# matt-suncy/symbols-from-video

Hardware: AMD Instinct MI355X
Metric: frames/sec (enc+binarise+dec fwd+bwd), batch 256x256, 1/2/4/8 MI355X (higher is better)
Workload: dtype bf16; 1 GPU; percep_RBVAE fused train step (batch gather from the HBM-resident latent table + fwd+bwd+losses+Adam), item [16,2,8,4,32,32] per GPU = 256 frames/step/GPU (latents of 256x256 frames), latent 32, 4-layer LSTMs, dropout on; parallelism=dp1, graph=True, dist_world_size=1, schedule=one HIP graph per step, devices_visible=1, graphs_captured=1, launcher=torch.distributed.run or self-spawned ranks

## Files before the change

include/rbvae_hip.h:

```cpp
#ifndef RBVAE_HIP_H
#define RBVAE_HIP_H

#include <stddef.h>
#include <stdint.h>

#ifdef __cplusplus
extern "C" {
#endif

#define RBVAE_OK 0
#define RBVAE_E_INVALID (-1)
#define RBVAE_E_LAUNCH (-2)
#define RBVAE_E_UNSUPPORTED (-3)

#define RBVAE_F32 0
#define RBVAE_BF16 1

int rbvae_version(void);
int rbvae_counter_add(unsigned long long* counter, unsigned long long inc, void* stream);
const char* rbvae_last_error(void);

int rbvae_binarize_kl_fwd(const float* h, const float* U, float* y_soft, float* z, float* kl_mean,
                          int rows, int L, float tau, float noise_ratio, float noise_eps, int hard,
                          float kl_p, float kl_eps, int kl_clamp, unsigned long long seed,
// ... 78 lines not shown

int rbvae_pack3(int dtype, const float* in, void* out, int d0, int d1, int d2, long s0, long s1, long s2,
                void* stream);
int rbvae_permute_reduce(const float* in, int nslab, long slab_stride, float* out, int d0, int d1, int d2, long s0,
                         long s1, long s2, float scale, int accumulate, void* stream);
int rbvae_cast_pad(int dtype, const float* in, void* out, int rows, int L, int Lpad, void* stream);
int rbvae_reduce_rows(const float* ws, int rows, int C, float* out, float scale, int accumulate, void* stream);
int rbvae_colsum_partial(int dtype, const void* X, int P, int C, int ld, float* ws, void* stream);
size_t rbvae_colsum_ws_floats(int P, int C);
int rbvae_colsum(int dtype, const void* X, int P, int C, int ld, float* out, float* ws, float scale, int accumulate,
                 void* stream);

int rbvae_run_jobs(const void* jobs_dev, int njobs, int blocks_per_job, void* stream);
int rbvae_job_block_map(const long* rows_host, int njobs, int max_blocks_per_job, int* map_host, int map_capacity);
int rbvae_run_jobs_sized(const void* jobs_dev, const void* block_map_dev, int total_blocks, void* stream);

int rbvae_im2col(int dtype, const float* src, long sn, long sc, long sh, long sw, int N, int C, int IH, int IW,
                 int OH, int OW, int KH, int KW, int stride, int pad, int Kpad, void* col, void* stream);
int rbvae_conv_first_fused_ok(int dtype, int Cin, int IH, int IW, int Nout, int N);
int rbvae_conv_first_fused(int dtype, const float* x, int fd1, int fd2, long fs0, long fs1, long fs2, const void* W,
                           const float* bias, const void* zero_page, void* col, void* out, int N, int Cin, int IH, int IW,
                           int Nout, int ldo, int relu, int drop_mode, float drop_p, float scale, unsigned long long seed,
                           const unsigned long long* seed_dev, void* stream);
int rbvae_deconv_last_dgrad_blocks(int dtype, int Cout, int OH, int OW, int C1, int N);
int rbvae_deconv_last_dgrad_fused(int dtype, const float* dpre, const void* W, const void* zero_page, void* col,
                                  const void* gate, void* out, int N, int Cout, int OH, int OW, int C1, int ldo, float scale,
                                  float* colsum_ws, void* stream);

int rbvae_wgrad_first_blocks(int dtype, int Cin, int IH, int IW, int Nout, int N);
int rbvae_wgrad_first(int dtype, int mode, const float* x, int fd1, int fd2, long fs0, long fs1, long fs2, const void* dY,
// ... 131 lines not shown
```

symbols-from-video_amd/_lib.py:

```python
import ctypes
import os
import re

import torch

HERE = os.path.dirname(os.path.abspath(__file__))
HEADER = os.path.join(os.path.dirname(HERE), "include", "rbvae_hip.h")
LIB_PATH = os.environ.get("RBVAE_LIB") or os.path.join(HERE, "librbvae_hip.so")

E_INVALID, E_LAUNCH, E_UNSUPPORTED = -1, -2, -3

_CTYPES = {
    "int": ctypes.c_int, "long": ctypes.c_long, "float": ctypes.c_float, "size_t": ctypes.c_size_t,
    "unsigned long long": ctypes.c_ulonglong, "unsigned": ctypes.c_uint, "double": ctypes.c_double,
}


def parse_header(path=HEADER):
    src = open(path).read()
    src = re.sub(r"/\*.*?\*/", "", src, flags=re.S)
    src = re.sub(r"//[^\n]*", "", src)
    protos = {}
    for m in re.finditer(r"\b(int|size_t|const char\*)\s+(rbvae_\w+)\s*\(([^)]*)\)\s*;", src):
        ret, name, args = m.group(1), m.group(2), m.group(3).strip()
        parsed = []
        if args and args != "void":
            for a in args.split(","):
                a = " ".join(a.split())
                if "*" in a:
                    parsed.append((ctypes.c_void_p, a.split("*")[-1].strip()))
                else:
                    ty, nm = a.rsplit(" ", 1)
                    parsed.append((_CTYPES[ty.replace("const ", "")], nm))
        restype = {"int": ctypes.c_int, "size_t": ctypes.c_size_t, "const char*": ctypes.c_char_p}[ret]
        protos[name] = (restype, parsed)
    return protos


_lib = None
_protos = None


def lib():
    global _lib, _protos
    if _lib is None:
        if not os.path.exists(LIB_PATH):
            raise RuntimeError(
                f"{LIB_PATH} is missing: build it with `python -c 'import __graft_entry__ as g; g.build()'` "
                "(hipcc, gfx950). There is no CPU or PyTorch fallback for the RBVAE hot path.")
        l = ctypes.CDLL(LIB_PATH)
        _protos = parse_header()
        for name, (restype, args) in _protos.items():
            fn = getattr(l, name)
            fn.restype = restype
            fn.argtypes = [t for t, _ in args]
        _lib = l
    return _lib


def _ptr(x):
    if x is None:
        return None
    if isinstance(x, torch.Tensor):
        return x.data_ptr()
    return x


def stream_ptr():
    return torch.cuda.current_stream().cuda_stream


def call(name, *args):
# ... 52 lines not shown
```

symbols-from-video_amd/csrc/jobs.hip:

```cpp
#include "common.h"

namespace rbvae {

struct Job {
    long type;
    const float* src;
    void* dst;
    long d0, d1, d2;
    long s0, s1, s2;
    long nslab, slab;
    long dtype;
    long accumulate;
    float scale;
    int fast;
    long inner;
    void* dst2;
};
static_assert(sizeof(Job) == 16 * 8, "job table stride");

struct AdamCtx {
    float* w; const float* g; float* m; float* v;
    const float* hyper;
    float one_m_b1, b2, one_m_b2, eps, gscale, pad_;
};
static_assert(sizeof(AdamCtx) == 8 * 8, "adam context layout (8 x int64 on the host side)");

__device__ __forceinline__ float adam_value(float w, float g, float& m, float& v, const AdamCtx& c, float step_size,
                                            float bc2_sqrt) {
    return adam_update(w, g, m, v, c.one_m_b1, c.b2, c.one_m_b2, c.eps, c.gscale, step_size, bc2_sqrt);
}
__device__ __forceinline__ float adam_at(const AdamCtx& c, long off, float step_size, float bc2_sqrt) {
    float m = c.m[off], v = c.v[off];
    const float w = adam_value(c.w[off], c.g[off], m, v, c, step_size, bc2_sqrt);
    c.m[off] = m; c.v[off] = v; c.w[off] = w;
    return w;
}

#ifndef CPK_CIB
#define CPK_CIB 64
#endif
constexpr int CPK_MAXROW = 2304;
constexpr int CPK_LDS_BYTES = 16 * (CPK_MAXROW + 8);
template <typename T>
__device__ __forceinline__ void conv_pack_rows(const Job& j, unsigned char* lds_raw, unsigned bidx, unsigned nblk) {
    constexpr unsigned NCO = 16 / sizeof(T), NV = 16 / sizeof(T);
    typedef __attribute__((ext_vector_type(4))) unsigned u32x4;
    T* tile = (T*)lds_raw;
    const unsigned Co = (unsigned)j.d0, Ci = (unsigned)j.d1, kk = (unsigned)j.d2;
    unsigned cib = (CPK_MAXROW / kk) / NV * NV;
    if (cib > Ci) cib = Ci;
    if (cib > CPK_CIB && Ci % CPK_CIB == 0) cib = CPK_CIB;
    const unsigned ncb = (Ci + cib - 1) / cib, ngr = (Co + NCO - 1) / NCO;
    const unsigned pitch = CPK_MAXROW + 8;
    T* wf = (T*)j.dst;
    T* wd = (T*)j.dst2;
    const bool vec_ok = (Ci % NV == 0) && (Co % NCO == 0) && ((cib * kk) % 4 == 0) && ((Ci * kk) % 4 == 0);
    const AdamCtx* actx = (const AdamCtx*)j.inner;
    float step_size = 0.f, bc2_sqrt = 1.f;
    if (actx) { step_size = actx->hyper[0]; bc2_sqrt = actx->hyper[1]; }
    for (unsigned b = bidx; b < ngr * ncb; b += nblk) {
        const unsigned co0 = (b / ncb) * NCO, ci0 = (b % ncb) * cib;
        const unsigned cn = min(cib, Ci - ci0), row = cn * kk;
        __syncthreads();
        if (vec_ok && actx) {
            const unsigned r4 = row / 4, tot = NCO * r4;
            constexpr unsigned AB = 3;
            for (unsigned i0 = threadIdx.x; i0 < tot; i0 += AB * 256) {
                float4 w4[AB], g4[AB], m4[AB], v4[AB];
                long off[AB];
#pragma unroll
                for (unsigned u = 0; u < AB; ++u) {
                    const unsigned i = i0 + u * 256, ic = i < tot ? i : 0;
                    const unsigned r = ic / r4, q = ic - r * r4;
                    off[u] = (j.src - actx->w) + ((long)(co0 + r) * Ci + ci0) * kk + 4 * q;
                    w4[u] = *(const float4*)(actx->w + off[u]); g4[u] = *(const float4*)(actx->g + off[u]);
                    m4[u] = *(const float4*)(actx->m + off[u]); v4[u] = *(const float4*)(actx->v + off[u]);
                }
#pragma unroll
                for (unsigned u = 0; u < AB; ++u) {
                    const unsigned i = i0 + u * 256;
                    if (i < tot) {
                        float4 w = w4[u], m = m4[u], v = v4[u];
                        w.x = adam_value(w.x, g4[u].x, m.x, v.x, *actx, step_size, bc2_sqrt);
                        w.y = adam_value(w.y, g4[u].y, m.y, v.y, *actx, step_size, bc2_sqrt);
                        w.z = adam_value(w.z, g4[u].z, m.z, v.z, *actx, step_size, bc2_sqrt);
                        w.w = adam_value(w.w, g4[u].w, m.w, v.w, *actx, step_size, bc2_sqrt);
                        *(float4*)(actx->w + off[u]) = w; *(float4*)(actx->m + off[u]) = m; *(float4*)(actx->v + off[u]) = v;
                        const unsigned r = i / r4, q = i - r * r4;
                        T* d = tile + r * pitch + 4 * q;
                        Elem<T>::store(d, w.x); Elem<T>::store(d + 1, w.y); Elem<T>::store(d + 2, w.z); Elem<T>::store(d + 3, w.w);
                    }
                }
            }
        } else if (vec_ok) {
            const unsigned r4 = row / 4, tot = NCO * r4;
            constexpr unsigned LB = 9;
            for (unsigned i0 = threadIdx.x; i0 < tot; i0 += LB * 256) {
                float4 v[LB];
#pragma unroll
                for (unsigned u = 0; u < LB; ++u) {
                    const unsigned i = i0 + u * 256, ic = i < tot ? i : 0;
                    const unsigned r = ic / r4, q = ic - r * r4;
                    v[u] = *(const float4*)(j.src + ((size_t)(co0 + r) * Ci + ci0) * kk + 4 * q);
                }
#pragma unroll
                for (unsigned u = 0; u < LB; ++u) {
                    const unsigned i = i0 + u * 256;
                    if (i < tot) {
// ... 33 lines not shown
                *(u32x4*)(wd + ((size_t)(ci0 + c) * kk + tp) * Co + co0) = *(const u32x4*)v;
            }
        } else {
            for (unsigned i = threadIdx.x; i < NCO * row; i += 256) {
                const unsigned r = i / row, e = i - r * row, c = e / kk, tp = e - c * kk;
                if (co0 + r < Co) {
                    const T v = tile[r * pitch + e];
                    wf[((size_t)(co0 + r) * kk + tp) * Ci + ci0 + c] = v;
                    wd[((size_t)(ci0 + c) * kk + tp) * Co + co0 + r] = v;
                }
            }
        }
    }
}

constexpr int CRD_CI = 256, CRD_MAXKK = 16, CRD_ACC = CRD_CI * CRD_MAXKK / 4 / 256;
__device__ __forceinline__ void conv_reduce_rows(const Job& j, float* tile, unsigned bidx, unsigned nblk) {
#if defined(JOBS_ABL_ONE_SLAB) && !defined(RBVAE_ABLATION)
#error "JOBS_ABL_ONE_SLAB gives wrong sums (timing ablation): define RBVAE_ABLATION to confirm"
#endif
#ifdef JOBS_ABL_ONE_SLAB
    const unsigned Co = (unsigned)j.d0, Ci = (unsigned)j.d1, kk = (unsigned)j.d2, ns = 1;
#else
    const unsigned Co = (unsigned)j.d0, Ci = (unsigned)j.d1, kk = (unsigned)j.d2, ns = (unsigned)j.nslab;
#endif
    const unsigned ncb = (Ci + CRD_CI - 1) / CRD_CI;
    float* out = (float*)j.dst;
    for (unsigned b = bidx; b < Co * ncb; b += nblk) {
        const unsigned co = b / ncb, ci0 = (b % ncb) * CRD_CI;
        const unsigned cn = min((unsigned)CRD_CI, Ci - ci0);
        const unsigned c4 = cn / 4, nch = kk * c4, pitch = cn + 1;
        float4 acc[CRD_ACC];
#pragma unroll
        for (int a = 0; a < CRD_ACC; ++a) acc[a] = make_float4(0.f, 0.f, 0.f, 0.f);
        const float* base = j.src + ((size_t)co * kk) * Ci + ci0;
        unsigned off[CRD_ACC];
        const int na = (int)((nch + 255) / 256);
#pragma unroll
        for (int a = 0; a < CRD_ACC; ++a) {
            const unsigned i = threadIdx.x + a * 256;
            const unsigned ic = i < nch ? i : 0, tp = ic / c4, q = ic - tp * c4;
            off[a] = tp * Ci + 4 * q;
        }
        unsigned k = 0;
        if (na == 1) {
            for (; k + 8 <= ns; k += 8) {
                float4 v[8];
#pragma unroll
                for (int s8 = 0; s8 < 8; ++s8) v[s8] = *(const float4*)(base + (size_t)(k + s8) * j.slab + off[0]);
#pragma unroll
                for (int s8 = 0; s8 < 8; ++s8) { acc[0].x += v[s8].x; acc[0].y += v[s8].y; acc[0].z += v[s8].z; acc[0].w += v[s8].w; }
            }
        }
        for (; k + 2 <= ns; k += 2) {
            float4 v[2][CRD_ACC];
#pragma unroll
            for (int s4 = 0; s4 < 2; ++s4)
#pragma unroll
                for (int a = 0; a < CRD_ACC; ++a)
                    if (a < na) v[s4][a] = *(const float4*)(base + (size_t)(k + s4) * j.slab + off[a]);
#pragma unroll
            for (int s4 = 0; s4 < 2; ++s4)
#pragma unroll
                for (int a = 0; a < CRD_ACC; ++a)
                    if (a < na) { acc[a].x += v[s4][a].x; acc[a].y += v[s4][a].y; acc[a].z += v[s4][a].z; acc[a].w += v[s4][a].w; }
        }
        for (; k < ns; ++k) {
            const float* p = base + (size_t)k * j.slab;
            float4 v[CRD_ACC];
#pragma unroll
            for (int a = 0; a < CRD_ACC; ++a)
                if (a < na) v[a] = *(const float4*)(p + off[a]);
#pragma unroll
            for (int a = 0; a < CRD_ACC; ++a)
                if (a < na) { acc[a].x += v[a].x; acc[a].y += v[a].y; acc[a].z += v[a].z; acc[a].w += v[a].w; }
        }
        __syncthreads();
#pragma unroll
        for (int a = 0; a < CRD_ACC; ++a) {
            const unsigned i = threadIdx.x + a * 256;
            if (i < nch) {
                const unsigned tp = i / c4, q = i - tp * c4;
                float* d = tile + tp * pitch + 4 * q;
                d[0] = acc[a].x * j.scale; d[1] = acc[a].y * j.scale; d[2] = acc[a].z * j.scale; d[3] = acc[a].w * j.scale;
            }
        }
        __syncthreads();
        float* orow = out + ((size_t)co * Ci + ci0) * kk;
        const unsigned n4 = cn * kk / 4;
        for (unsigned i = threadIdx.x; i < n4; i += 256) {
            float4 o;
            float* op = (float*)&o;
#pragma unroll
            for (unsigned u = 0; u < 4; ++u) {
                const unsigned e = 4 * i + u, c = e / kk, tp = e - c * kk;
                op[u] = tile[tp * pitch + c];
            }
            if (j.accumulate) {
                const float4 w = *(const float4*)(orow + 4 * i);
                o.x += w.x; o.y += w.y; o.z += w.z; o.w += w.w;
            }
            *(float4*)(orow + 4 * i) = o;
        }
    }
}

__global__ __launch_bounds__(256) void run_jobs_k(const Job* __restrict__ jobs, const int4* __restrict__ map) {
    __shared__ __attribute__((aligned(16))) unsigned char lds_raw[CPK_LDS_BYTES];
    static_assert(CPK_LDS_BYTES >= (int)sizeof(float) * CRD_MAXKK * (CRD_CI + 1), "the reduce tile fits the pack tile");
    static_assert(CPK_LDS_BYTES >= 256 * 16, "the wide row reduction's tree fits");
    unsigned bidx = blockIdx.x, nblk = gridDim.x, jidx = blockIdx.y;
    if (map) {
        const int4 m = map[blockIdx.x];
        jidx = (unsigned)m.x; bidx = (unsigned)m.y; nblk = (unsigned)m.z;
    }
    const Job j = jobs[jidx];
    if (j.type == 3) {
        if (j.dtype == RBVAE_F32) conv_pack_rows<float>(j, lds_raw, bidx, nblk); else conv_pack_rows<bf16_t>(j, lds_raw, bidx, nblk);
        return;
    }
    if (j.type == 4) {
        conv_reduce_rows(j, (float*)lds_raw, bidx, nblk);
        return;
    }
    if (j.type == 6 || j.type == 7) {
        const AdamCtx c = *(const AdamCtx*)j.inner;
        const float step_size = c.hyper[0], bc2_sqrt = c.hyper[1];
        const unsigned d1 = (unsigned)j.d1, d2 = (unsigned)j.d2;
        const long n = j.d0 * j.d1 * j.d2, base = j.src - c.w;
        const int t1 = (int)(j.dtype & 255), t2 = (int)((j.dtype >> 8) & 255);
#ifndef JOBS_TILED_ADAM
#define JOBS_TILED_ADAM 1
#endif
        if (JOBS_TILED_ADAM && j.type == 6 && n >= (1l << 20)) {
            const long a0 = j.s0, a1 = j.s1, a2 = j.s2, c0 = j.nslab, c1 = j.slab, c2 = j.accumulate;
            const int fA = a0 == 1 ? 0 : (a1 == 1 ? 1 : 2);
            const int fB = !j.dst2 ? fA : (c0 == 1 ? 0 : (c1 == 1 ? 1 : 2));
            if (fA != 2 || fB != 2) {
                const unsigned D0 = (unsigned)j.d0;
                unsigned T0, T1, T2;
                if (fA != 2 && fB != 2 && fA != fB) { T2 = 16; T0 = fB == 0 ? 32 : 16; T1 = fB == 1 ? 32 : 16; }
                else { const int f = fA != 2 ? fA : fB; T2 = 32; T0 = f == 0 ? 32 : 8; T1 = f == 1 ? 32 : 8; }
                T0 = min(T0, D0); T1 = min(T1, d1); T2 = min(T2, d2);
                const unsigned nt0 = (D0 + T0 - 1) / T0, nt1 = (d1 + T1 - 1) / T1, nt2 = (d2 + T2 - 1) / T2;
                const unsigned pitch = T2 + 1, tel = T0 * T1 * T2;
                float* tile = (float*)lds_raw;
                for (unsigned t = bidx; t < nt0 * nt1 * nt2; t += nblk) {
                    const unsigned b2 = (t % nt2) * T2, b1 = ((t / nt2) % nt1) * T1, b0 = (t / (nt2 * nt1)) * T0;
                    for (unsigned e0 = threadIdx.x; e0 < tel; e0 += 1024) {
                        long off[4]; unsigned li[4]; bool ok[4];
                        float pw[4], pg[4], pm[4], pv[4];
#pragma unroll
                        for (int u = 0; u < 4; ++u) {
                            const unsigned e = e0 + 256 * u;
                            const unsigned l2 = e % T2, l1 = (e / T2) % T1, l0 = e / (T2 * T1);
                            ok[u] = e < tel && b0 + l0 < D0 && b1 + l1 < d1 && b2 + l2 < d2;
                            off[u] = base + ((long)(b0 + l0) * d1 + (b1 + l1)) * d2 + (b2 + l2);
                            li[u] = (l0 * T1 + l1) * pitch + l2;
// ... 52 lines not shown
        const long b = counter ? (long)(counter[0] % (unsigned long long)nb) : 0;
        const float4* table = (const float4*)j.src;
        float4* out = (float4*)j.dst;
        for (long r = bidx; r < rows; r += nblk) {
            long src = plan[b * rows + r];
            if (src < 0 || src >= table_rows) src = 0;
            for (long i = threadIdx.x; i < vec; i += 256) out[r * vec + i] = table[src * vec + i];
        }
        return;
    }
    const unsigned d0 = (unsigned)j.d0, d1 = (unsigned)j.d1, d2 = (unsigned)j.d2;
    const unsigned n = d0 * d1 * d2;
    if (bidx * (j.type == 2 ? 4u : 256u) >= n) return;
    if (j.type == 2) {
        const unsigned nsl = (unsigned)j.nslab, slb = (unsigned)j.slab;
        if (nsl >= 1024 && (n & 3) == 0 && (slb & 3) == 0 && ((size_t)j.src & 15) == 0) {
            float4* red = (float4*)lds_raw;
            float* out = (float*)j.dst;
            for (unsigned cb = bidx; cb < n / 4; cb += nblk) {
                float4 a = make_float4(0.f, 0.f, 0.f, 0.f);
                const float* col = j.src + 4 * cb;
                unsigned k = threadIdx.x;
                for (; k + 7 * 256 < nsl; k += 8 * 256) {
                    float4 v[8];
#pragma unroll
                    for (int u = 0; u < 8; ++u) v[u] = *(const float4*)(col + (size_t)(k + u * 256) * slb);
#pragma unroll
                    for (int u = 0; u < 8; ++u) { a.x += v[u].x; a.y += v[u].y; a.z += v[u].z; a.w += v[u].w; }
                }
                for (; k < nsl; k += 256) {
                    const float4 v = *(const float4*)(col + (size_t)k * slb);
// ... 93 lines not shown
        const unsigned fv = i % ef, r = i / ef;
        const unsigned mid = r % em, slow = r / em;
        const unsigned i0 = f == 0 ? fv : slow;
        const unsigned i1 = f == 1 ? fv : (f == 0 ? slow : mid);
        const unsigned i2 = f == 2 ? fv : mid;
        const size_t lin = ((size_t)i0 * d1 + i1) * d2 + i2;
        const size_t so = i0 * (size_t)j.s0 + i1 * (size_t)j.s1 + i2 * (size_t)j.s2;
        if (j.type == 0) {
            if (j.dtype == RBVAE_F32) ((float*)j.dst)[so] = j.src[lin];
            else ((bf16_t*)j.dst)[so] = f32_to_bf16(j.src[lin]);
        } else {
            const float* p = j.src + so;
            float a = 0.f;
            const unsigned ns = (unsigned)j.nslab;
            unsigned k = 0;
            for (; k + 16 <= ns; k += 16) {
                float v[16];
#pragma unroll
                for (int u = 0; u < 16; ++u) v[u] = p[(size_t)(k + u) * j.slab];
#pragma unroll
                for (int u = 0; u < 16; ++u) a += v[u];
            }
            for (; k + 4 <= ns; k += 4) {
                const float v0 = p[(size_t)k * j.slab], v1 = p[(size_t)(k + 1) * j.slab];
                const float v2 = p[(size_t)(k + 2) * j.slab], v3 = p[(size_t)(k + 3) * j.slab];
                a = (((a + v0) + v1) + v2) + v3;
            }
            for (; k < ns; ++k) a += p[(size_t)k * j.slab];
            a *= j.scale;
            float* out = (float*)j.dst;
            out[lin] = j.accumulate ? out[lin] + a : a;
        }
    }
}

}

using namespace rbvae;

extern "C" int rbvae_run_jobs(const void* jobs_dev, int njobs, int blocks_per_job, void* stream) {
    RBVAE_CHECK_ARG(jobs_dev && njobs > 0 && blocks_per_job > 0, "run_jobs: bad arguments");
    RBVAE_CHECK_ARG(njobs <= 65535, "run_jobs: too many jobs");
    hipLaunchKernelGGL(run_jobs_k, dim3(blocks_per_job, njobs), dim3(256), 0, (hipStream_t)stream, (const Job*)jobs_dev,
                       (const int4*)nullptr);
    RBVAE_CHECK_LAUNCH("run_jobs");
    return RBVAE_OK;
}

static long job_blocks_of(const long* r) {
    const long type = r[0], d0 = r[3], d1 = r[4], d2 = r[5], n = d0 * d1 * d2;
    const long dtype = r[11];
    if (type == 3) {
        const long es = (dtype & 255) == RBVAE_F32 ? 4 : 2, nco = 16 / es, nv = 16 / es, kk = d2;
        long cib = (CPK_MAXROW / kk) / nv * nv;
        if (cib > d1) cib = d1;
        if (cib > CPK_CIB && d1 % CPK_CIB == 0) cib = CPK_CIB;
        return ((d0 + nco - 1) / nco) * ((d1 + cib - 1) / cib);
    }
    if (type == 4) return d0 * ((d1 + CRD_CI - 1) / CRD_CI);
    if (type == 5) return d0;
    if (type == 6 || type == 7) {
        if (type == 6 && n >= (1l << 20)) {
            const long a0 = r[6], a1 = r[7], c0 = r[9], c1 = r[10];
            const int fA = a0 == 1 ? 0 : (a1 == 1 ? 1 : 2);
            const int fB = !r[15] ? fA : (c0 == 1 ? 0 : (c1 == 1 ? 1 : 2));
            if (fA != 2 || fB != 2) {
                long T0, T1, T2;
                if (fA != 2 && fB != 2 && fA != fB) { T2 = 16; T0 = fB == 0 ? 32 : 16; T1 = fB == 1 ? 32 : 16; }
                else { const int f = fA != 2 ? fA : fB; T2 = 32; T0 = f == 0 ? 32 : 8; T1 = f == 1 ? 32 : 8; }
                if (T0 > d0) T0 = d0;
                if (T1 > d1) T1 = d1;
                if (T2 > d2) T2 = d2;
                return ((d0 + T0 - 1) / T0) * ((d1 + T1 - 1) / T1) * ((d2 + T2 - 1) / T2);
            }
        }
        return (n + 255) / 256;
    }
    if (type == 2) return (n + 3) / 4;
    if (r[14]) return (d0 * d1 + 255) / 256;
    return (n + 255) / 256;
}

extern "C" int rbvae_job_block_map(const long* rows_host, int njobs, int max_blocks_per_job, int* map_host, int map_capacity) {
    if (!rows_host || njobs <= 0 || max_blocks_per_job <= 0) return fail(RBVAE_E_INVALID, "job_block_map: bad arguments");
    long total = 0;
    for (int j = 0; j < njobs; ++j) {
        long nb = job_blocks_of(rows_host + 16l * j);
        if (nb < 1) nb = 1;
        if (nb > max_blocks_per_job) nb = max_blocks_per_job;
        if (map_host) {
            if (total + nb > map_capacity) return fail(RBVAE_E_INVALID, "job_block_map: map of %d entries is too small", map_capacity);
            for (long b = 0; b < nb; ++b) {
                int* m = map_host + 4 * (total + b);
                m[0] = j; m[1] = (int)b; m[2] = (int)nb; m[3] = 0;
            }
        }
        total += nb;
    }
    if (total >= (1l << 31)) return fail(RBVAE_E_INVALID, "job_block_map: too many workgroups");
    return (int)total;
}

extern "C" int rbvae_run_jobs_sized(const void* jobs_dev, const void* block_map_dev, int total_blocks, void* stream) {
    RBVAE_CHECK_ARG(jobs_dev && block_map_dev && total_blocks > 0, "run_jobs_sized: bad arguments");
    RBVAE_CHECK_ARG((uintptr_t)block_map_dev % 16 == 0, "run_jobs_sized: the block map must be 16-byte aligned");
    hipLaunchKernelGGL(run_jobs_k, dim3(total_blocks), dim3(256), 0, (hipStream_t)stream, (const Job*)jobs_dev,
                       (const int4*)block_map_dev);
    RBVAE_CHECK_LAUNCH("run_jobs_sized");
    return RBVAE_OK;
}
```

symbols-from-video_amd/engine.py:

```python
from __future__ import annotations

import math
import os
from dataclasses import dataclass
from typing import Dict, List, Optional, Sequence, Tuple

import torch

from . import _lib as L

F32, BF16 = 0, 1


@dataclass(frozen=True)
class Variant:
    name: str
    channels: Tuple[int, int, int]
    kernel: int
    lstm_layers: int
    dropout: float
    noise_ratio_arg: bool
    eps: float
    simple_order: bool
    default_hw: Tuple[int, int]
# ... 132 lines not shown

    def signature(self):
        return tuple(tuple(r) for r in self.rows)


def job_block_map(rows, device, cap):
    import numpy as np
    arr = np.ascontiguousarray(np.array(rows, dtype=np.int64).reshape(len(rows), 16))
    total = L.query("rbvae_job_block_map", arr.ctypes.data, len(rows), cap, None, 0)
    if total <= 0:
        raise RuntimeError("rbvae_job_block_map: " + L.lib().rbvae_last_error().decode())
    m = np.empty(4 * total, dtype=np.int32)
    if L.query("rbvae_job_block_map", arr.ctypes.data, len(rows), cap, m.ctypes.data, total) != total:
        raise RuntimeError("rbvae_job_block_map: " + L.lib().rbvae_last_error().decode())
    return torch.from_numpy(m).to(device), total


class Saved:
    __slots__ = ("N", "S", "T", "hw", "train", "tau", "tau_dev", "hard", "col1", "x_in", "fm_in", "a1", "a2", "a3", "e", "hs_enc", "hp_enc",
                 "acts_enc", "cs_enc", "y", "z", "hs_dec", "hp_dec", "acts_dec", "cs_dec", "ds_pad", "f", "d1", "d2",
                 "xr", "gate_scale", "dpre3", "b3_parts")


class Engine:
    def __init__(self, variant: str, in_ch: int, out_ch: int, latent: int, hw: Tuple[int, int],
                 dtype: str = "f32", device: Optional[torch.device] = None):
        if variant not in VARIANTS:
            raise ValueError(f"unknown variant {variant!r}")
        if dtype not in ("f32", "bf16"):
            raise ValueError("dtype must be 'f32' or 'bf16'")
# ... 24 lines not shown
        self.Lp = _ru(latent, self.ke)
        self.zero = torch.zeros(256, dtype=torch.uint8, device=self.device)
        self._cls_conv = conv_classes(k)
        self._cls_dgrad, self._ncls_dgrad = dgrad_classes(k)
        self._desc_cache: Dict[Tuple, object] = {}
        self._idx_cache: Dict[Tuple, torch.Tensor] = {}
        self.seed_dev = None
        self._pack_tab: Dict = {}
        self._bufs: Dict = {}
        self._bwd_tab: Dict = {}
        self._jobs: Optional[JobList] = None
        self._wg_cus = 256
        self.last_wgrad_kernel = None
        self._job_blocks = 256
        self.sized_jobs = 2
        self._side: Optional[torch.cuda.Stream] = None
        self.overlap = True
        self._ks_small = 3
        self.fc_gemm = True
        self.deconv_halo = True
        self._dh_min_wgs = 1024
        self.conv_s2_halo = True
        self._cs_min_wgs = 512
        self._cs_max_waste = 1.15
        self.wgrad_halo = True
        self._wh_min_steps = 8
        self._wh_max_tiles = 2
        self.wgrad_row = True
        self._wr_min_steps = 4
        self._wr_slab_mb = 64
# ... 29 lines not shown
        self.WfcT = z(self.F3, self.Lp)
        self.Wdfc = z(self.F3, self.Lp)
        self.WdfcT = z(self.latent, self.F3)
        self.bdfc = torch.zeros(self.F3, dtype=torch.float32, device=self.device)
        self.V1f, self.V1d = z(c3, kk, c2), z(c2, kk, c3)
        self.V2f, self.V2d = z(c2, kk, c1), z(c1, kk, c2)
        self.V3p = z(self.NY, c1)
        self.V3f = z(c1, self.K3)
        nl, Ld = self.v.lstm_layers, self.latent
        self.wT_enc = torch.zeros(nl, 2, Ld, 4 * Ld, dtype=torch.float32, device=self.device)
        self.wT_dec = torch.zeros(nl, 2, Ld, 4 * Ld, dtype=torch.float32, device=self.device)

    def _register_table(self, tab: torch.Tensor, rows):
        if not hasattr(self, "_table_maps"):
            self._table_maps = {}
        self._table_maps[tab.data_ptr()] = job_block_map(rows, self.device, self._job_blocks) + (tab,)

    def run_table(self, tab: torch.Tensor, n: int, kind: int = 2):
        m = getattr(self, "_table_maps", {}).get(tab.data_ptr())
        if m is None or self.sized_jobs < kind:
            L.call("rbvae_run_jobs", tab, n, self._job_blocks)
        else:
            L.call("rbvae_run_jobs_sized", tab, m[0], m[1])

    def pack(self, flat: torch.Tensor):
        key = flat.data_ptr()
        tab = self._pack_tab.get(key)
        if tab is None:
            jl = self._pack_jobs(flat)
            tab = (jl.upload(self.device), len(jl.rows), jl)
            self._register_table(tab[0], jl.rows)
            self._pack_tab[key] = tab
        self.run_table(tab[0], tab[1])

    def update_jobs(self, flat, gflat, m, v, hyper, betas, eps, gscale, extra_rows=None, part=None):
        import struct
        key = ("update", flat.data_ptr(), gflat.data_ptr(), m.data_ptr(), v.data_ptr(), hyper.data_ptr(), tuple(betas),
               float(eps), float(gscale), tuple(map(tuple, extra_rows)) if extra_rows else None, part)
# ... 717 lines not shown
```

Measured before the change: 571,000 frames/s.

## Size job-kernel LDS per table, add walk scheduler and deeper reduce loads

The job runner kernel now takes dynamic LDS sized to the largest need of the jobs in each table, so low-LDS tables can run more workgroups per CU. The conv-pack CI block shrinks to 32 with a pitch derived from the block. The slab reductions now keep more loads in flight through templated groups. An optional persistent 'walk' launcher balances items across groups by byte cost; it is off by default via an environment variable. Smaller pack tiles mean more blocks and more per-block overhead, and the deeper unrolls raise register pressure.

```diff
diff --git a/include/rbvae_hip.h b/include/rbvae_hip.h
--- a/include/rbvae_hip.h
+++ b/include/rbvae_hip.h
@@ -116,6 +116,12 @@
 int rbvae_run_jobs(const void* jobs_dev, int njobs, int blocks_per_job, void* stream);
 int rbvae_job_block_map(const long* rows_host, int njobs, int max_blocks_per_job, int* map_host, int map_capacity);
 int rbvae_run_jobs_sized(const void* jobs_dev, const void* block_map_dev, int total_blocks, void* stream);
+int rbvae_job_lds_bytes(const long* rows_host, int njobs);
+int rbvae_run_jobs_sized_lds(const void* jobs_dev, const void* block_map_dev, int total_blocks, int lds_bytes, void* stream);
+int rbvae_job_walk_map(const long* rows_host, int njobs, int max_blocks_per_job, int groups, int* items_host, int items_capacity,
+                       int* bounds_host);
+int rbvae_run_jobs_walk(const void* jobs_dev, int njobs, const void* items_dev, int nitems, const void* bounds_dev, int groups,
+                        int lds_bytes, void* stream);
 
 int rbvae_im2col(int dtype, const float* src, long sn, long sc, long sh, long sw, int N, int C, int IH, int IW,
                  int OH, int OW, int KH, int KW, int stride, int pad, int Kpad, void* col, void* stream);
diff --git a/symbols-from-video_amd/_lib.py b/symbols-from-video_amd/_lib.py
--- a/symbols-from-video_amd/_lib.py
+++ b/symbols-from-video_amd/_lib.py
@@ -37,6 +37,8 @@
     return protos
 
 
+OPTIONAL_IN_AB = ("rbvae_job_lds_bytes", "rbvae_run_jobs_sized_lds", "rbvae_job_walk_map", "rbvae_run_jobs_walk")
+
 _lib = None
 _protos = None
 
@@ -51,11 +53,17 @@
         l = ctypes.CDLL(LIB_PATH)
         _protos = parse_header()
         for name, (restype, args) in _protos.items():
+            if os.environ.get("RBVAE_LIB") and name in OPTIONAL_IN_AB and not hasattr(l, name):
+                continue
             fn = getattr(l, name)
             fn.restype = restype
             fn.argtypes = [t for t, _ in args]
         _lib = l
     return _lib
+
+
+def has(name):
+    return hasattr(lib(), name)
 
 
 def _ptr(x):
diff --git a/symbols-from-video_amd/csrc/jobs.hip b/symbols-from-video_amd/csrc/jobs.hip
--- a/symbols-from-video_amd/csrc/jobs.hip
+++ b/symbols-from-video_amd/csrc/jobs.hip
@@ -37,21 +37,70 @@
 }
 
 #ifndef CPK_CIB
-#define CPK_CIB 64
+#define CPK_CIB 32
 #endif
 constexpr int CPK_MAXROW = 2304;
 constexpr int CPK_LDS_BYTES = 16 * (CPK_MAXROW + 8);
+#ifndef CPK_AB
+#define CPK_AB 3
+#endif
+
+__host__ __device__ inline unsigned cpk_cib(unsigned Ci, unsigned kk, unsigned nv) {
+    unsigned cib = (CPK_MAXROW / kk) / nv * nv;
+    if (cib > Ci) cib = Ci;
+    if (cib > CPK_CIB && Ci % CPK_CIB == 0) cib = CPK_CIB;
+    return cib;
+}
+__host__ __device__ inline long cpk_blocks(long Co, long Ci, long kk, long nv) {
+    const long cib = cpk_cib((unsigned)Ci, (unsigned)kk, (unsigned)nv);
+    return ((Co + nv - 1) / nv) * ((Ci + cib - 1) / cib);
+}
+__host__ __device__ inline unsigned cpk_lds_bytes(unsigned Ci, unsigned kk, unsigned nv) { return 16u * (cpk_cib(Ci, kk, nv) * kk + 8u); }
+
+template <typename T, unsigned AB>
+__device__ __forceinline__ void cpk_adam_in(const Job& j, const AdamCtx* actx, float step_size, float bc2_sqrt, T* tile,
+                                            unsigned pitch, unsigned co0, unsigned ci0, unsigned Ci, unsigned kk, unsigned r4,
+                                            unsigned tot) {
+    for (unsigned i0 = threadIdx.x; i0 < tot; i0 += AB * 256) {
+        float4 w4[AB], g4[AB], m4[AB], v4[AB];
+        long off[AB];
+#pragma unroll
+        for (unsigned u = 0; u < AB; ++u) {
+            const unsigned i = i0 + u * 256, ic = i < tot ? i : 0;
+            const unsigned r = ic / r4, q = ic - r * r4;
+            off[u] = (j.src - actx->w) + ((long)(co0 + r) * Ci + ci0) * kk + 4 * q;
+            w4[u] = *(const float4*)(actx->w + off[u]); g4[u] = *(const float4*)(actx->g + off[u]);
+            m4[u] = *(const float4*)(actx->m + off[u]); v4[u] = *(const float4*)(actx->v + off[u]);
+        }
+#pragma unroll
+        for (unsigned u = 0; u < AB; ++u) {
+            const unsigned i = i0 + u * 256;
+            if (i < tot) {
+                float4 w = w4[u], m = m4[u], v = v4[u];
+                w.x = adam_value(w.x, g4[u].x, m.x, v.x, *actx, step_size, bc2_sqrt);
+                w.y = adam_value(w.y, g4[u].y, m.y, v.y, *actx, step_size, bc2_sqrt);
+                w.z = adam_value(w.z, g4[u].z, m.z, v.z, *actx, step_size, bc2_sqrt);
+                w.w = adam_value(w.w, g4[u].w, m.w, v.w, *actx, step_size, bc2_sqrt);
+                *(float4*)(actx->w + off[u]) = w; *(float4*)(actx->m + off[u]) = m; *(float4*)(actx->v + off[u]) = v;
+                const unsigned r = i / r4, q = i - r * r4;
+                T* d = tile + r * pitch + 4 * q;
+                Elem<T>::store(d, w.x); Elem<T>::store(d + 1, w.y); Elem<T>::store(d + 2, w.z); Elem<T>::store(d + 3, w.w);
+            }
+        }
+    }
+}
+
 template <typename T>
-__device__ __forceinline__ void conv_pack_rows(const Job& j, unsigned char* lds_raw, unsigned bidx, unsigned nblk) {
+__device__ __forceinline__ void conv_pack_rows(const Job& j, unsigned char* lds_raw, unsigned lds_bytes, unsigned bidx,
+                                               unsigned nblk) {
     constexpr unsigned NCO = 16 / sizeof(T), NV = 16 / sizeof(T);
     typedef __attribute__((ext_vector_type(4))) unsigned u32x4;
     T* tile = (T*)lds_raw;
     const unsigned Co = (unsigned)j.d0, Ci = (unsigned)j.d1, kk = (unsigned)j.d2;
-    unsigned cib = (CPK_MAXROW / kk) / NV * NV;
-    if (cib > Ci) cib = Ci;
-    if (cib > CPK_CIB && Ci % CPK_CIB == 0) cib = CPK_CIB;
+    const unsigned cib = cpk_cib(Ci, kk, NV);
     const unsigned ncb = (Ci + cib - 1) / cib, ngr = (Co + NCO - 1) / NCO;
-    const unsigned pitch = CPK_MAXROW + 8;
+    const unsigned pitch = cib * kk + 8;
+    if (cpk_lds_bytes(Ci, kk, NV) > lds_bytes) return;
     T* wf = (T*)j.dst;
     T* wd = (T*)j.dst2;
     const bool vec_ok = (Ci % NV == 0) && (Co % NCO == 0) && ((cib * kk) % 4 == 0) && ((Ci * kk) % 4 == 0);
@@ -64,34 +113,8 @@
         __syncthreads();
         if (vec_ok && actx) {
             const unsigned r4 = row / 4, tot = NCO * r4;
-            constexpr unsigned AB = 3;
-            for (unsigned i0 = threadIdx.x; i0 < tot; i0 += AB * 256) {
-                float4 w4[AB], g4[AB], m4[AB], v4[AB];
-                long off[AB];
-#pragma unroll
-                for (unsigned u = 0; u < AB; ++u) {
-                    const unsigned i = i0 + u * 256, ic = i < tot ? i : 0;
-                    const unsigned r = ic / r4, q = ic - r * r4;
-                    off[u] = (j.src - actx->w) + ((long)(co0 + r) * Ci + ci0) * kk + 4 * q;
-                    w4[u] = *(const float4*)(actx->w + off[u]); g4[u] = *(const float4*)(actx->g + off[u]);
-                    m4[u] = *(const float4*)(actx->m + off[u]); v4[u] = *(const float4*)(actx->v + off[u]);
-                }
-#pragma unroll
-                for (unsigned u = 0; u < AB; ++u) {
-                    const unsigned i = i0 + u * 256;
-                    if (i < tot) {
-                        float4 w = w4[u], m = m4[u], v = v4[u];
-                        w.x = adam_value(w.x, g4[u].x, m.x, v.x, *actx, step_size, bc2_sqrt);
-                        w.y = adam_value(w.y, g4[u].y, m.y, v.y, *actx, step_size, bc2_sqrt);
-                        w.z = adam_value(w.z, g4[u].z, m.z, v.z, *actx, step_size, bc2_sqrt);
-                        w.w = adam_value(w.w, g4[u].w, m.w, v.w, *actx, step_size, bc2_sqrt);
-                        *(float4*)(actx->w + off[u]) = w; *(float4*)(actx->m + off[u]) = m; *(float4*)(actx->v + off[u]) = v;
-                        const unsigned r = i / r4, q = i - r * r4;
-                        T* d = tile + r * pitch + 4 * q;
-                        Elem<T>::store(d, w.x); Elem<T>::store(d + 1, w.y); Elem<T>::store(d + 2, w.z); Elem<T>::store(d + 3, w.w);
-                    }
-                }
-            }
+            if (CPK_AB > 3 && tot > 3 * 256) cpk_adam_in<T, CPK_AB>(j, actx, step_size, bc2_sqrt, tile, pitch, co0, ci0, Ci, kk, r4, tot);
+            else cpk_adam_in<T, 3>(j, actx, step_size, bc2_sqrt, tile, pitch, co0, ci0, Ci, kk, r4, tot);
         } else if (vec_ok) {
             const unsigned r4 = row / 4, tot = NCO * r4;
             constexpr unsigned LB = 9;
@@ -155,8 +178,40 @@
     }
 }
 
-constexpr int CRD_CI = 256, CRD_MAXKK = 16, CRD_ACC = CRD_CI * CRD_MAXKK / 4 / 256;
-__device__ __forceinline__ void conv_reduce_rows(const Job& j, float* tile, unsigned bidx, unsigned nblk) {
+#ifndef PRD_INFLIGHT
+#define PRD_INFLIGHT 32
+#endif
+#ifndef CRD_CIB
+#define CRD_CIB 64
+#endif
+constexpr int CRD_CI = CRD_CIB, CRD_MAXKK = 16, CRD_ACC = (CRD_CI * CRD_MAXKK / 4 + 255) / 256;
+#ifndef CRD_INFLIGHT
+#define CRD_INFLIGHT 16
+#endif
+__host__ __device__ inline long crd_blocks(long Co, long Ci) { return Co * ((Ci + CRD_CI - 1) / CRD_CI); }
+__host__ __device__ inline unsigned crd_lds_bytes(unsigned Ci, unsigned kk) { return kk * ((Ci < (unsigned)CRD_CI ? Ci : (unsigned)CRD_CI) + 1u) * 4u; }
+
+template <int NA>
+__device__ __forceinline__ void crd_sum_slabs(const float* base, long slab, unsigned ns, const unsigned* off, float4* acc) {
+    constexpr int GS = CRD_INFLIGHT / NA;
+    for (unsigned k = 0; k < ns; k += GS) {
+        float4 v[GS][NA];
+#pragma unroll
+        for (int s = 0; s < GS; ++s)
+            if (k + s < ns) {
+#pragma unroll
+                for (int a = 0; a < NA; ++a) v[s][a] = *(const float4*)(base + (size_t)(k + s) * slab + off[a]);
+            }
+#pragma unroll
+        for (int s = 0; s < GS; ++s)
+            if (k + s < ns) {
+#pragma unroll
+                for (int a = 0; a < NA; ++a) { acc[a].x += v[s][a].x; acc[a].y += v[s][a].y; acc[a].z += v[s][a].z; acc[a].w += v[s][a].w; }
+            }
+    }
+}
+
+__device__ __forceinline__ void conv_reduce_rows(const Job& j, float* tile, unsigned lds_bytes, unsigned bidx, unsigned nblk) {
 #if defined(JOBS_ABL_ONE_SLAB) && !defined(RBVAE_ABLATION)
 #error "JOBS_ABL_ONE_SLAB gives wrong sums (timing ablation): define RBVAE_ABLATION to confirm"
 #endif
@@ -167,6 +222,7 @@
 #endif
     const unsigned ncb = (Ci + CRD_CI - 1) / CRD_CI;
     float* out = (float*)j.dst;
+    if (kk > (unsigned)CRD_MAXKK || crd_lds_bytes(Ci, kk) > lds_bytes) return;
     for (unsigned b = bidx; b < Co * ncb; b += nblk) {
         const unsigned co = b / ncb, ci0 = (b % ncb) * CRD_CI;
         const unsigned cn = min((unsigned)CRD_CI, Ci - ci0);
@@ -183,39 +239,10 @@
             const unsigned ic = i < nch ? i : 0, tp = ic / c4, q = ic - tp * c4;
             off[a] = tp * Ci + 4 * q;
         }
-        unsigned k = 0;
-        if (na == 1) {
-            for (; k + 8 <= ns; k += 8) {
-                float4 v[8];
-#pragma unroll
-                for (int s8 = 0; s8 < 8; ++s8) v[s8] = *(const float4*)(base + (size_t)(k + s8) * j.slab + off[0]);
-#pragma unroll
-                for (int s8 = 0; s8 < 8; ++s8) { acc[0].x += v[s8].x; acc[0].y += v[s8].y; acc[0].z += v[s8].z; acc[0].w += v[s8].w; }
-            }
-        }
-        for (; k + 2 <= ns; k += 2) {
-            float4 v[2][CRD_ACC];
-#pragma unroll
-            for (int s4 = 0; s4 < 2; ++s4)
-#pragma unroll
-                for (int a = 0; a < CRD_ACC; ++a)
-                    if (a < na) v[s4][a] = *(const float4*)(base + (size_t)(k + s4) * j.slab + off[a]);
-#pragma unroll
-            for (int s4 = 0; s4 < 2; ++s4)
-#pragma unroll
-                for (int a = 0; a < CRD_ACC; ++a)
-                    if (a < na) { acc[a].x += v[s4][a].x; acc[a].y += v[s4][a].y; acc[a].z += v[s4][a].z; acc[a].w += v[s4][a].w; }
-        }
-        for (; k < ns; ++k) {
-            const float* p = base + (size_t)k * j.slab;
-            float4 v[CRD_ACC];
-#pragma unroll
-            for (int a = 0; a < CRD_ACC; ++a)
-                if (a < na) v[a] = *(const float4*)(p + off[a]);
-#pragma unroll
-            for (int a = 0; a < CRD_ACC; ++a)
-                if (a < na) { acc[a].x += v[a].x; acc[a].y += v[a].y; acc[a].z += v[a].z; acc[a].w += v[a].w; }
-        }
+        if (na == 1) crd_sum_slabs<1>(base, j.slab, ns, off, acc);
+        else if (CRD_ACC >= 2 && na == 2) crd_sum_slabs<CRD_ACC >= 2 ? 2 : 1>(base, j.slab, ns, off, acc);
+        else if (CRD_ACC >= 3 && na == 3) crd_sum_slabs<CRD_ACC >= 3 ? 3 : 1>(base, j.slab, ns, off, acc);
+        else if (CRD_ACC >= 4) crd_sum_slabs<CRD_ACC >= 4 ? 4 : 1>(base, j.slab, ns, off, acc);
         __syncthreads();
 #pragma unroll
         for (int a = 0; a < CRD_ACC; ++a) {
@@ -246,22 +273,31 @@
     }
 }
 
-__global__ __launch_bounds__(256) void run_jobs_k(const Job* __restrict__ jobs, const int4* __restrict__ map) {
-    __shared__ __attribute__((aligned(16))) unsigned char lds_raw[CPK_LDS_BYTES];
-    static_assert(CPK_LDS_BYTES >= (int)sizeof(float) * CRD_MAXKK * (CRD_CI + 1), "the reduce tile fits the pack tile");
-    static_assert(CPK_LDS_BYTES >= 256 * 16, "the wide row reduction's tree fits");
-    unsigned bidx = blockIdx.x, nblk = gridDim.x, jidx = blockIdx.y;
-    if (map) {
-        const int4 m = map[blockIdx.x];
-        jidx = (unsigned)m.x; bidx = (unsigned)m.y; nblk = (unsigned)m.z;
-    }
-    const Job j = jobs[jidx];
+#ifndef JOBS_TILED_ADAM
+#define JOBS_TILED_ADAM 1
+#endif
+__host__ __device__ inline bool adam_tile_dims(long type, long n, long a0, long a1, long c0, long c1, bool has2, unsigned D0,
+                                               unsigned d1, unsigned d2, int& fA, int& fB, unsigned& T0, unsigned& T1, unsigned& T2) {
+    fA = a0 == 1 ? 0 : (a1 == 1 ? 1 : 2);
+    fB = !has2 ? fA : (c0 == 1 ? 0 : (c1 == 1 ? 1 : 2));
+    if (!(JOBS_TILED_ADAM && type == 6 && n >= (1l << 20)) || (fA == 2 && fB == 2)) return false;
+    if (fA != 2 && fB != 2 && fA != fB) { T2 = 16; T0 = fB == 0 ? 32 : 16; T1 = fB == 1 ? 32 : 16; }
+    else { const int f = fA != 2 ? fA : fB; T2 = 32; T0 = f == 0 ? 32 : 8; T1 = f == 1 ? 32 : 8; }
+    T0 = T0 < D0 ? T0 : D0; T1 = T1 < d1 ? T1 : d1; T2 = T2 < d2 ? T2 : d2;
+    return true;
+}
+__host__ __device__ inline bool rows_wide(unsigned nsl, unsigned n, unsigned slb, const void* src) {
+    return nsl >= 1024 && (n & 3) == 0 && (slb & 3) == 0 && ((size_t)src & 15) == 0;
+}
+
+__device__ __forceinline__ void run_piece(const Job& j, unsigned char* lds_raw, unsigned lds_bytes, unsigned bidx, unsigned nblk) {
     if (j.type == 3) {
-        if (j.dtype == RBVAE_F32) conv_pack_rows<float>(j, lds_raw, bidx, nblk); else conv_pack_rows<bf16_t>(j, lds_raw, bidx, nblk);
+        if (j.dtype == RBVAE_F32) conv_pack_rows<float>(j, lds_raw, lds_bytes, bidx, nblk);
+        else conv_pack_rows<bf16_t>(j, lds_raw, lds_bytes, bidx, nblk);
         return;
     }
     if (j.type == 4) {
-        conv_reduce_rows(j, (float*)lds_raw, bidx, nblk);
+        conv_reduce_rows(j, (float*)lds_raw, lds_bytes, bidx, nblk);
         return;
     }
     if (j.type == 6 || j.type == 7) {
@@ -270,19 +306,13 @@
         const unsigned d1 = (unsigned)j.d1, d2 = (unsigned)j.d2;
         const long n = j.d0 * j.d1 * j.d2, base = j.src - c.w;
         const int t1 = (int)(j.dtype & 255), t2 = (int)((j.dtype >> 8) & 255);
-#ifndef JOBS_TILED_ADAM
-#define JOBS_TILED_ADAM 1
-#endif
-        if (JOBS_TILED_ADAM && j.type == 6 && n >= (1l << 20)) {
+        {
             const long a0 = j.s0, a1 = j.s1, a2 = j.s2, c0 = j.nslab, c1 = j.slab, c2 = j.accumulate;
-            const int fA = a0 == 1 ? 0 : (a1 == 1 ? 1 : 2);
-            const int fB = !j.dst2 ? fA : (c0 == 1 ? 0 : (c1 == 1 ? 1 : 2));
-            if (fA != 2 || fB != 2) {
-                const unsigned D0 = (unsigned)j.d0;
-                unsigned T0, T1, T2;
-                if (fA != 2 && fB != 2 && fA != fB) { T2 = 16; T0 = fB == 0 ? 32 : 16; T1 = fB == 1 ? 32 : 16; }
-                else { const int f = fA != 2 ? fA : fB; T2 = 32; T0 = f == 0 ? 32 : 8; T1 = f == 1 ? 32 : 8; }
-                T0 = min(T0, D0); T1 = min(T1, d1); T2 = min(T2, d2);
+            const unsigned D0 = (unsigned)j.d0;
+            int fA, fB;
+            unsigned T0, T1, T2;
+            if (adam_tile_dims(j.type, n, a0, a1, c0, c1, j.dst2 != nullptr, D0, d1, d2, fA, fB, T0, T1, T2)) {
+                if (T0 * T1 * (T2 + 1) * 4 > lds_bytes) return;
                 const unsigned nt0 = (D0 + T0 - 1) / T0, nt1 = (d1 + T1 - 1) / T1, nt2 = (d2 + T2 - 1) / T2;
                 const unsigned pitch = T2 + 1, tel = T0 * T1 * T2;
                 float* tile = (float*)lds_raw;
@@ -365,7 +395,8 @@
     if (bidx * (j.type == 2 ? 4u : 256u) >= n) return;
     if (j.type == 2) {
         const unsigned nsl = (unsigned)j.nslab, slb = (unsigned)j.slab;
-        if (nsl >= 1024 && (n & 3) == 0 && (slb & 3) == 0 && ((size_t)j.src & 15) == 0) {
+        if (rows_wide(nsl, n, slb, j.src)) {
+            if (lds_bytes < 256 * 16) return;
             float4* red = (float4*)lds_raw;
             float* out = (float*)j.dst;
             for (unsigned cb = bidx; cb < n / 4; cb += nblk) {
@@ -489,6 +520,15 @@
             float a = 0.f;
             const unsigned ns = (unsigned)j.nslab;
             unsigned k = 0;
+#if PRD_INFLIGHT >= 32
+            for (; k + 32 <= ns; k += 32) {
+                float v[32];
+#pragma unroll
+                for (int u = 0; u < 32; ++u) v[u] = p[(size_t)(k + u) * j.slab];
+#pragma unroll
+                for (int u = 0; u < 32; ++u) a += v[u];
+            }
+#endif
             for (; k + 16 <= ns; k += 16) {
                 float v[16];
 #pragma unroll
@@ -509,6 +549,33 @@
     }
 }
 
+
+__global__ __launch_bounds__(256) void run_jobs_k(const Job* __restrict__ jobs, const int4* __restrict__ map, unsigned lds_bytes) {
+    extern __shared__ __attribute__((aligned(16))) unsigned char lds_raw[];
+    static_assert(CPK_LDS_BYTES >= (int)sizeof(float) * CRD_MAXKK * (CRD_CI + 1), "the reduce tile fits the pack tile");
+    static_assert(CPK_LDS_BYTES >= 256 * 16, "the wide row reduction's tree fits");
+    static_assert(CPK_LDS_BYTES >= 32 * 8 * 33 * 4 && CPK_LDS_BYTES >= 32 * 16 * 17 * 4, "the tiled update's tile fits");
+    unsigned bidx = blockIdx.x, nblk = gridDim.x, jidx = blockIdx.y;
+    if (map) {
+        const int4 m = map[blockIdx.x];
+        jidx = (unsigned)m.x; bidx = (unsigned)m.y; nblk = (unsigned)m.z;
+    }
+    const Job j = jobs[jidx];
+    run_piece(j, lds_raw, lds_bytes, bidx, nblk);
+}
+
+__global__ __launch_bounds__(256) void run_jobs_walk_k(const Job* __restrict__ jobs, unsigned njobs, const int4* __restrict__ items,
+                                                       unsigned nitems, const int* __restrict__ bounds, unsigned lds_bytes) {
+    extern __shared__ __attribute__((aligned(16))) unsigned char lds_raw[];
+    const unsigned a = min((unsigned)bounds[blockIdx.x], nitems), b = min((unsigned)bounds[blockIdx.x + 1], nitems);
+    for (unsigned it = a; it < b; ++it) {
+        const int4 m = items[it];
+        const Job j = jobs[min((unsigned)m.x, njobs - 1)];
+        run_piece(j, lds_raw, lds_bytes, (unsigned)m.y, max((unsigned)m.z, 1u));
+        __syncthreads();
+    }
+}
+
 }
 
 using namespace rbvae;
@@ -516,44 +583,61 @@
 extern "C" int rbvae_run_jobs(const void* jobs_dev, int njobs, int blocks_per_job, void* stream) {
     RBVAE_CHECK_ARG(jobs_dev && njobs > 0 && blocks_per_job > 0, "run_jobs: bad arguments");
     RBVAE_CHECK_ARG(njobs <= 65535, "run_jobs: too many jobs");
-    hipLaunchKernelGGL(run_jobs_k, dim3(blocks_per_job, njobs), dim3(256), 0, (hipStream_t)stream, (const Job*)jobs_dev,
-                       (const int4*)nullptr);
+    hipLaunchKernelGGL(run_jobs_k, dim3(blocks_per_job, njobs), dim3(256), CPK_LDS_BYTES, (hipStream_t)stream, (const Job*)jobs_dev,
+                       (const int4*)nullptr, (unsigned)CPK_LDS_BYTES);
     RBVAE_CHECK_LAUNCH("run_jobs");
     return RBVAE_OK;
 }
 
 static long job_blocks_of(const long* r) {
     const long type = r[0], d0 = r[3], d1 = r[4], d2 = r[5], n = d0 * d1 * d2;
-    const long dtype = r[11];
-    if (type == 3) {
-        const long es = (dtype & 255) == RBVAE_F32 ? 4 : 2, nco = 16 / es, nv = 16 / es, kk = d2;
-        long cib = (CPK_MAXROW / kk) / nv * nv;
-        if (cib > d1) cib = d1;
-        if (cib > CPK_CIB && d1 % CPK_CIB == 0) cib = CPK_CIB;
-        return ((d0 + nco - 1) / nco) * ((d1 + cib - 1) / cib);
-    }
-    if (type == 4) return d0 * ((d1 + CRD_CI - 1) / CRD_CI);
+    if (type == 3) return cpk_blocks(d0, d1, d2, r[11] == RBVAE_F32 ? 4 : 8);
+    if (type == 4) return crd_blocks(d0, d1);
     if (type == 5) return d0;
     if (type == 6 || type == 7) {
-        if (type == 6 && n >= (1l << 20)) {
-            const long a0 = r[6], a1 = r[7], c0 = r[9], c1 = r[10];
-            const int fA = a0 == 1 ? 0 : (a1 == 1 ? 1 : 2);
-            const int fB = !r[15] ? fA : (c0 == 1 ? 0 : (c1 == 1 ? 1 : 2));
-            if (fA != 2 || fB != 2) {
-                long T0, T1, T2;
-                if (fA != 2 && fB != 2 && fA != fB) { T2 = 16; T0 = fB == 0 ? 32 : 16; T1 = fB == 1 ? 32 : 16; }
-                else { const int f = fA != 2 ? fA : fB; T2 = 32; T0 = f == 0 ? 32 : 8; T1 = f == 1 ? 32 : 8; }
-                if (T0 > d0) T0 = d0;
-                if (T1 > d1) T1 = d1;
-                if (T2 > d2) T2 = d2;
-                return ((d0 + T0 - 1) / T0) * ((d1 + T1 - 1) / T1) * ((d2 + T2 - 1) / T2);
-            }
-        }
+        int fA, fB;
+        unsigned T0, T1, T2;
+        if (adam_tile_dims(type, n, r[6], r[7], r[9], r[10], r[15] != 0, (unsigned)d0, (unsigned)d1, (unsigned)d2, fA, fB, T0, T1, T2))
+            return ((d0 + T0 - 1) / T0) * ((d1 + T1 - 1) / T1) * ((d2 + T2 - 1) / T2);
         return (n + 255) / 256;
     }
     if (type == 2) return (n + 3) / 4;
     if (r[14]) return (d0 * d1 + 255) / 256;
     return (n + 255) / 256;
+}
+
+static long job_lds_of(const long* r) {
+    const long type = r[0], d0 = r[3], d1 = r[4], d2 = r[5], n = d0 * d1 * d2;
+    if (d0 <= 0 || d1 <= 0 || d2 <= 0) return 0;
+    if (type == 3) return d2 > 16 ? 0 : cpk_lds_bytes((unsigned)d1, (unsigned)d2, r[11] == RBVAE_F32 ? 4 : 8);
+    if (type == 4) return d2 > CRD_MAXKK ? 0 : crd_lds_bytes((unsigned)d1, (unsigned)d2);
+    if (type == 6) {
+        int fA, fB;
+        unsigned T0, T1, T2;
+        if (adam_tile_dims(type, n, r[6], r[7], r[9], r[10], r[15] != 0, (unsigned)d0, (unsigned)d1, (unsigned)d2, fA, fB, T0, T1, T2))
+            return (long)T0 * T1 * (T2 + 1) * 4;
+        return 0;
+    }
+    if (type == 2) return rows_wide((unsigned)r[9], (unsigned)n, (unsigned)r[10], (const void*)r[1]) ? 256 * 16 : 0;
+    return 0;
+}
+
+static long job_bytes_of(const long* r) {
+    const long type = r[0], d0 = r[3], d1 = r[4], d2 = r[5], n = d0 * d1 * d2, ns = r[9] > 0 ? r[9] : 1;
+    if (type == 3) return n * (r[14] ? 32 : 8);
+    if (type == 4 || type == 1) return n * 4 * (ns + 1);
+    if (type == 2) return n * 4 * ns;
+    if (type == 5) return d0 * d2 * 32;
+    if (type == 6 || type == 7) return n * 32;
+    return n * 8;
+}
+
+extern "C" int rbvae_job_lds_bytes(const long* rows_host, int njobs) {
+    if (!rows_host || njobs <= 0) return fail(RBVAE_E_INVALID, "job_lds_bytes: bad arguments");
+    long need = 0;
+    for (int j = 0; j < njobs; ++j) { const long b = job_lds_of(rows_host + 16l * j); if (b > need) need = b; }
+    if (need > CPK_LDS_BYTES) return fail(RBVAE_E_INVALID, "job_lds_bytes: a job needs %ld bytes of LDS (at most %d)", need, CPK_LDS_BYTES);
+    return (int)need;
 }
 
 extern "C" int rbvae_job_block_map(const long* rows_host, int njobs, int max_blocks_per_job, int* map_host, int map_capacity) {
@@ -576,11 +660,60 @@
     return (int)total;
 }
 
-extern "C" int rbvae_run_jobs_sized(const void* jobs_dev, const void* block_map_dev, int total_blocks, void* stream) {
+static int run_jobs_sized(const void* jobs_dev, const void* block_map_dev, int total_blocks, int lds_bytes, void* stream) {
     RBVAE_CHECK_ARG(jobs_dev && block_map_dev && total_blocks > 0, "run_jobs_sized: bad arguments");
     RBVAE_CHECK_ARG((uintptr_t)block_map_dev % 16 == 0, "run_jobs_sized: the block map must be 16-byte aligned");
-    hipLaunchKernelGGL(run_jobs_k, dim3(total_blocks), dim3(256), 0, (hipStream_t)stream, (const Job*)jobs_dev,
-                       (const int4*)block_map_dev);
+    RBVAE_CHECK_ARG(lds_bytes >= 0 && lds_bytes <= CPK_LDS_BYTES, "run_jobs_sized: LDS bytes out of range");
+    hipLaunchKernelGGL(run_jobs_k, dim3(total_blocks), dim3(256), (size_t)lds_bytes, (hipStream_t)stream, (const Job*)jobs_dev,
+                       (const int4*)block_map_dev, (unsigned)lds_bytes);
     RBVAE_CHECK_LAUNCH("run_jobs_sized");
     return RBVAE_OK;
 }
+
+extern "C" int rbvae_run_jobs_sized(const void* jobs_dev, const void* block_map_dev, int total_blocks, void* stream) {
+    return run_jobs_sized(jobs_dev, block_map_dev, total_blocks, CPK_LDS_BYTES, stream);
+}
+
+extern "C" int rbvae_run_jobs_sized_lds(const void* jobs_dev, const void* block_map_dev, int total_blocks, int lds_bytes, void* stream) {
+    return run_jobs_sized(jobs_dev, block_map_dev, total_blocks, lds_bytes, stream);
+}
+
+extern "C" int rbvae_job_walk_map(const long* rows_host, int njobs, int max_blocks_per_job, int groups, int* items_host,
+                                  int items_capacity, int* bounds_host) {
+    if (!rows_host || njobs <= 0 || max_blocks_per_job <= 0 || groups <= 0) return fail(RBVAE_E_INVALID, "job_walk_map: bad arguments");
+    const int total = rbvae_job_block_map(rows_host, njobs, max_blocks_per_job, items_host, items_capacity);
+    if (total < 0 || !items_host) return total;
+    if (!bounds_host) return fail(RBVAE_E_INVALID, "job_walk_map: no room for the range bounds");
+    auto cost = [&](int i) {
+        const long* r = rows_host + 16l * items_host[4 * i];
+        return job_bytes_of(r) / items_host[4 * i + 2] + 4096;
+    };
+    double sum = 0;
+    for (int i = 0; i < total; ++i) sum += (double)cost(i);
+    double cum = 0;
+    int g = 0;
+    bounds_host[0] = 0;
+    for (int i = 0; i < total; ++i) {
+        const double c = (double)cost(i);
+        int gi = (int)((cum + 0.5 * c) * groups / sum);
+        if (gi >= groups) gi = groups - 1;
+        while (g < gi) bounds_host[++g] = i;
+        cum += c;
+    }
+    while (g < groups) bounds_host[++g] = total;
+    for (int k = 0; k < groups; ++k)
+        if (bounds_host[k] > bounds_host[k + 1] || bounds_host[k] < 0) return fail(RBVAE_E_INVALID, "job_walk_map: ranges out of order");
+    if (bounds_host[0] != 0 || bounds_host[groups] != total) return fail(RBVAE_E_INVALID, "job_walk_map: ranges do not cover the items");
+    return total;
+}
+
+extern "C" int rbvae_run_jobs_walk(const void* jobs_dev, int njobs, const void* items_dev, int nitems, const void* bounds_dev,
+                                   int groups, int lds_bytes, void* stream) {
+    RBVAE_CHECK_ARG(jobs_dev && items_dev && bounds_dev && njobs > 0 && nitems > 0 && groups > 0, "run_jobs_walk: bad arguments");
+    RBVAE_CHECK_ARG((uintptr_t)items_dev % 16 == 0, "run_jobs_walk: the item map must be 16-byte aligned");
+    RBVAE_CHECK_ARG(lds_bytes >= 0 && lds_bytes <= CPK_LDS_BYTES, "run_jobs_walk: LDS bytes out of range");
+    hipLaunchKernelGGL(run_jobs_walk_k, dim3(groups), dim3(256), (size_t)lds_bytes, (hipStream_t)stream, (const Job*)jobs_dev,
+                       (unsigned)njobs, (const int4*)items_dev, (unsigned)nitems, (const int*)bounds_dev, (unsigned)lds_bytes);
+    RBVAE_CHECK_LAUNCH("run_jobs_walk");
+    return RBVAE_OK;
+}
diff --git a/symbols-from-video_amd/engine.py b/symbols-from-video_amd/engine.py
--- a/symbols-from-video_amd/engine.py
+++ b/symbols-from-video_amd/engine.py
@@ -170,6 +170,27 @@
     if L.query("rbvae_job_block_map", arr.ctypes.data, len(rows), cap, m.ctypes.data, total) != total:
         raise RuntimeError("rbvae_job_block_map: " + L.lib().rbvae_last_error().decode())
     return torch.from_numpy(m).to(device), total
+
+
+def job_walk_bounds(rows, device, cap, groups):
+    import numpy as np
+    arr = np.ascontiguousarray(np.array(rows, dtype=np.int64).reshape(len(rows), 16))
+    total = L.query("rbvae_job_walk_map", arr.ctypes.data, len(rows), cap, groups, None, 0, None)
+    if total <= 0:
+        raise RuntimeError("rbvae_job_walk_map: " + L.lib().rbvae_last_error().decode())
+    items, bounds = np.empty(4 * total, dtype=np.int32), np.empty(groups + 1, dtype=np.int32)
+    if L.query("rbvae_job_walk_map", arr.ctypes.data, len(rows), cap, groups, items.ctypes.data, total, bounds.ctypes.data) != total:
+        raise RuntimeError("rbvae_job_walk_map: " + L.lib().rbvae_last_error().decode())
+    return torch.from_numpy(bounds).to(device)
+
+
+def job_lds_bytes(rows):
+    import numpy as np
+    arr = np.ascontiguousarray(np.array(rows, dtype=np.int64).reshape(len(rows), 16))
+    n = L.query("rbvae_job_lds_bytes", arr.ctypes.data, len(rows))
+    if n < 0:
+        raise RuntimeError("rbvae_job_lds_bytes: " + L.lib().rbvae_last_error().decode())
+    return n
 
 
 class Saved:
@@ -224,6 +245,8 @@
         self.last_wgrad_kernel = None
         self._job_blocks = 256
         self.sized_jobs = 2
+        self.walk_jobs = int(os.environ.get("RBVAE_WALK_JOBS", "0"))
+        self._walk_groups = 768
         self._side: Optional[torch.cuda.Stream] = None
         self.overlap = True
         self._ks_small = 3
@@ -283,14 +306,20 @@
     def _register_table(self, tab: torch.Tensor, rows):
         if not hasattr(self, "_table_maps"):
             self._table_maps = {}
-        self._table_maps[tab.data_ptr()] = job_block_map(rows, self.device, self._job_blocks) + (tab,)
+        lds = job_lds_bytes(rows) if L.has("rbvae_run_jobs_sized_lds") else None
+        bounds = job_walk_bounds(rows, self.device, self._job_blocks, self._walk_groups) if L.has("rbvae_run_jobs_walk") else None
+        self._table_maps[tab.data_ptr()] = job_block_map(rows, self.device, self._job_blocks) + (tab, lds, bounds)
 
     def run_table(self, tab: torch.Tensor, n: int, kind: int = 2):
         m = getattr(self, "_table_maps", {}).get(tab.data_ptr())
         if m is None or self.sized_jobs < kind:
             L.call("rbvae_run_jobs", tab, n, self._job_blocks)
-        else:
+        elif m[3] is None:
             L.call("rbvae_run_jobs_sized", tab, m[0], m[1])
+        elif self.walk_jobs >= kind and m[4] is not None:
+            L.call("rbvae_run_jobs_walk", tab, n, m[0], m[1], m[4], m[4].numel() - 1, m[3])
+        else:
+            L.call("rbvae_run_jobs_sized_lds", tab, m[0], m[1], m[3])
 
     def pack(self, flat: torch.Tensor):
         key = flat.data_ptr()
```

After: 570,500 frames/s. About the same (-0.1%).
